# Meeso1/nmmo

Hardware: AMD Instinct MI355X
Metric: agent-steps/sec (whole node), 128-agent envs at 1/2/4/8 MI355X (higher is better)
Workload: dtype int16

## Files before the change

nmmo_amd/csrc/flat_obs.hip:

```cpp
#include "agent_obs.h"

namespace nmmo {

#ifndef NMMO_FO_ABL
#define NMMO_FO_ABL 0
#endif
#ifndef NMMO_FO_STAMPS
#define NMMO_FO_STAMPS 0
#endif
#if NMMO_FO_STAMPS
constexpr int kFoStamps = 12;
__device__ uint64_t fo_stamp_buf[1 << 17][kFoStamps];
__device__ uint64_t fo_wave_buf[1 << 15][6];
#define FO_STAMP(k) fst[k] = __builtin_amdgcn_s_memtime()
#else
#define FO_STAMP(k) (void)0
#endif
#ifndef NMMO_FO_XCD
#define NMMO_FO_XCD 1
#endif
#ifndef NMMO_FO_TILE_SKIP
#define NMMO_FO_TILE_SKIP 0
#endif
#ifndef NMMO_FO_TASK_BATCH
#define NMMO_FO_TASK_BATCH 8
#endif
constexpr int kFoTaskBatch = NMMO_FO_TASK_BATCH;
constexpr int kFoStagedListings = 64;
constexpr int kFoChunks = 25;
static_assert(kFoChunks * 64 >= kMaskN + 2 && (kFoChunks - 1) * 64 < kMaskN, "mask chunks");
static_assert(kFlatId == kMaskN && kFlatTick == kMaskN + 1 && kFlatEntity == kMaskN + 2, "id, tick in the last chunk");
static_assert(kWireBuyLo / 64 == 1 && (kWireBuyLo + NMMO_MARKET_ROWS) / 64 == 17, "Buy.MarketItem: chunks 1 to 17");

constexpr int kFoVisw = (kNObs + 3) & ~3;
constexpr int kFoWinRowBytes = 16, kFoWinAgentBytes = 15 * kFoWinRowBytes;
constexpr size_t kFoWinBytes = (size_t)kAoAgents * kFoWinAgentBytes, kFoItemBytes = (size_t)kAoAgents * kInv * 8;
static_assert(F_COL == F_ROW + 1 && kAoPkBytes <= kFoWinBytes, "shared LDS regions");
__host__ __device__ constexpr bool fo_items_in_T(int S) {
  return (size_t)2 * ao_stride(S) * 2 >= kFoItemBytes && (F_ROW * ao_stride(S) * 2) % 8 == 0;
}
constexpr int kFoListPool = NMMO_MARKET_ROWS * 2 + kFoStagedListings * 8;
__host__ __device__ constexpr int fo_staged(int nm) {
  return nm < ((kFoListPool - ((2 * nm + 7) & ~7)) >> 3) ? nm : (kFoListPool - ((2 * nm + 7) & ~7)) >> 3;
}
static_assert(fo_staged(NMMO_MARKET_ROWS) == kFoStagedListings && fo_staged(256) == 256 && fo_staged(257) == 255 &&
                  fo_staged(0) == 0 && kFoListPool % 16 == 0, "listings' pool");
__host__ __device__ constexpr size_t fo_lds_bytes(int S) {
  return ao_columns_lds(S) + (size_t)kFoListPool +
         (size_t)kAoWaves * kFoVisw * 4 + kFoWinBytes + (fo_items_in_T(S) ? 0 : kFoItemBytes);
// ... 17 lines not shown
__device__ __forceinline__ uint64_t fo_shift(uint64_t lo, uint64_t hi) {
  if constexpr (kSh >= 64) {
    return 0ull;
  } else if constexpr (kSh > 0) {
    return lo << kSh;
  } else if constexpr (kSh == 0) {
    return lo;
  } else if constexpr (-kSh < 64) {
    return (lo >> (-kSh)) | (hi << (64 + kSh));
  } else if constexpr (-kSh < 128) {
    return hi >> (-kSh - 64);
  } else {
    return 0ull;
  }
}
template <int kK, int kC>
__device__ __forceinline__ uint64_t fo_sec(uint64_t lo, uint64_t hi) {
  constexpr int off = sec_flat(kK), n = kSecN[kK];
  if constexpr (off >= 64 * kC + 64 || off + n <= 64 * kC) return 0ull;
  else return fo_shift<off - 64 * kC>(lo, hi);
}
template <int kC>
__device__ __forceinline__ uint64_t fo_chunk(const AoSections& x) {
  return fo_sec<0, kC>(x.s0, 0ull) | fo_sec<1, kC>(x.s1[0], x.s1[1]) | fo_sec<3, kC>(x.s3, 0ull) |
         fo_sec<4, kC>(x.s4, 0ull) | fo_sec<5, kC>(x.s5[0], x.s5[1]) | fo_sec<6, kC>(x.s6[0], x.s6[1]) |
         fo_sec<7, kC>(x.s7[0], x.s7[1]) | fo_sec<8, kC>(x.s8, 0ull) | fo_sec<9, kC>(x.s9, 0ull) |
         fo_sec<10, kC>(x.s10[0], x.s10[1]) | fo_sec<11, kC>(x.s11, 0ull);
}
__device__ __forceinline__ float fo_bit(uint64_t m) { return __builtin_amdgcn_inverse_ballot_w64(m) ? 1.f : 0.f; }
__device__ __forceinline__ void fo_st(float* row, uint32_t idx, float v) {
  *reinterpret_cast<float*>(reinterpret_cast<char*>(row) + (idx << 2)) = v;
}

constexpr int kFoTail0 = (kWireBuyLo + NMMO_MARKET_ROWS) / 64;
__host__ __device__ constexpr int fo_slot(int c) { return c < 2 ? c : c - kFoTail0 + 2; }
static_assert(fo_slot(kFoChunks - 1) == 9 && kZext == 10 + 1 + 12, "tracked chunks | position | items");
struct FoImg {
  bool ext;
  uint32_t lo, hi;
  int j10;
  int nimg;
  int nst;
};
__device__ __forceinline__ uint64_t fo_prev(const FoImg& g, int slot) {
  return (uint64_t)(uint32_t)__builtin_amdgcn_readlane((int)g.lo, g.j10 + slot) |
         (uint64_t)(uint32_t)__builtin_amdgcn_readlane((int)g.hi, g.j10 + slot) << 32;
}
template <int kC>
__device__ __forceinline__ void fo_put(float* row, FoImg& g, uint64_t m, float aid, float tick) {
  constexpr int sl = fo_slot(kC);
  const int lane = ao_lane();
  const bool same = g.ext && m == fo_prev(g, sl);
  if constexpr (kC == kFoChunks - 1) {
    constexpr int n = kMaskN - 64 * kC;
    if (!same) {
      if (lane < n + 2) fo_st(row, 64 * kC + lane, lane < n ? fo_bit(m) : lane == n ? aid : tick);
      g.nst += n + 2;
    } else {
      if (lane == n + 1) fo_st(row, 64 * kC + lane, tick);
      g.nst += 1;
    }
  } else if (!same) {
    fo_st(row, 64 * kC + lane, fo_bit(m));
    g.nst += 64;
  }
  g.nimg = writelane<2 * sl>((int)(uint32_t)m, g.nimg);
  g.nimg = writelane<2 * sl + 1>((int)(uint32_t)(m >> 32), g.nimg);
}
template <int kC>
__device__ __forceinline__ void fo_tail_chunks(float* row, FoImg& g, const AoSections& x, uint64_t buy17, float aid,
                                               float tick) {
  if constexpr (kC < kFoChunks) {
    uint64_t m = fo_chunk<kC>(x);
    if constexpr (kC == kFoTail0) m |= buy17 | 1ull << ((kWireBuyLo + NMMO_MARKET_ROWS) & 63);
    fo_put<kC>(row, g, m, aid, tick);
    fo_tail_chunks<kC + 1>(row, g, x, buy17, aid, tick);
  }
}

constexpr int kFoPassRows = 16;
static_assert(kFoPassRows == 16 && kAoAgents / kAoWaves * kFoPassRows <= 64 && kInv <= kFoPassRows &&
                  kFoGather <= kFoPassRows, "a 16-lane group per agent");
constexpr int kFoBuyLane = 48;
struct FoPass {
  uint32_t lo, hi;
  uint64_t chg;
  uint64_t idiff;
};
template <int kSl>
__device__ __forceinline__ void fo_pass_chunks(const AoSections& x, int sl, uint64_t& m) {
  if constexpr (kSl < 10) {
    constexpr int c = kSl < 2 ? kSl : kSl - 2 + kFoTail0;
    static_assert(fo_slot(c) == kSl, "tracked chunk");
    const uint64_t mc = fo_chunk<c>(x);
    if (sl == kSl) m = mc;
    fo_pass_chunks<kSl + 1>(x, sl, m);
  }
}
template <bool kWrap>
__device__ __forceinline__ FoPass fo_mask_pass(const ObsParams& p, int e, int w, int abase, int nm, const int16_t* own,
                                               const uint32_t* visw, const uint8_t* wsb, const uint2* ist,
                                               const uint16_t* mpo, int my_nv, uint32_t my_rc, int my_prev, int my_alive,
                                               int my_task, uint64_t zvalid, uint64_t zextv, uint2 img, uint2 pinv) {
  constexpr int kPerWave = kAoAgents / kAoWaves;
  const bool combat = (p.systems & NMMO_SYS_COMBAT) != 0;
  const bool item = (p.systems & NMMO_SYS_ITEM) != 0;
  const bool exch = item && (p.systems & NMMO_SYS_EXCHANGE) != 0;
  const bool no_give = kWrap && (p.wflags & kWrapObsNoGive);
  const bool no_danger = kWrap && (p.wflags & kWrapObsNoDangerous);
  const int lane = lane_id(), P = p.P;
  const int gj = lane >> 4, gk = lane & 15, ga = abase + kAoWaves * gj, gla = w + kAoWaves * gj;
  const int grc = __shfl((int)my_rc, gj);
  const int gr = (int16_t)(grc & 0xFFFF), gc = grc >> 16;
  bool tgt = false, st = false;
  if (gk < __shfl(my_nv, gj)) ao_row_preds(visw[gj * kFoVisw + gk], ga, gr, gc, combat, no_danger, tgt, st);
  const uint64_t tb = __ballot(tgt), sb = __ballot(st);
  const uint2 it = gk < kInv ? ist[gla * kInv + gk] : make_uint2(0u, 0u);
  const uint64_t occ = __ballot(gk < kInv && it_type(it) != 0);
  const bool have = gk < __builtin_ctz(~((uint32_t)(occ >> (16 * gj)) & 0xFFFFu));
  const uint64_t bfr = __ballot(have && !it_equipped(it) && !it_price(it));
// ... 64 lines not shown
#pragma unroll
    for (int d = 0; d < 5; d++)
      if (!impassable((int)wa[(kVision + dir_dr(d)) * kFoWinRowBytes + kVision + dir_dc(d)])) b |= 1u << d;
    x.s8 = b;
  }
  uint64_t m = 0ull;
  fo_pass_chunks<0>(x, sl, m);
  uint64_t bw0 = 0ull, bw15 = 0ull;
  FoPass o;
  o.lo = img.x;
  o.hi = img.y;
  if (exch && nm > 0) {
    const uint32_t po0 = lane < nm ? mpo[lane] : 0u, po15 = 15 * 64 + lane < nm ? mpo[15 * 64 + lane] : 0u;
#pragma unroll
    for (int j = 0; j < kPerWave; j++) {
      const int a = abase + kAoWaves * j;
      const int gold = __builtin_amdgcn_readfirstlane((int)own[(w + kAoWaves * j) * kMirrorCols + F_GOLD]);
      const uint64_t b0 = __ballot(lane < nm && (int)(po0 & 255u) <= gold && (int)(po0 >> 8) != a);
      uint64_t b15 = 0ull;
      if (nm > 15 * 64) b15 = __ballot(15 * 64 + lane < nm && (int)(po15 & 255u) <= gold && (int)(po15 >> 8) != a);
      if (ja == j) bw0 = b0, bw15 = b15;
      if (lane == kFoBuyLane + j) o.lo = (uint32_t)b0, o.hi = (uint32_t)(b0 >> 32);
    }
  }
  if (sl == 1) m |= bw0 << (kWireBuyLo & 63);
  if (sl == 2) m |= bw15 >> (64 - (kWireBuyLo & 63)) | 1ull << ((kWireBuyLo + NMMO_MARKET_ROWS) & 63);
  const bool ext = (zextv >> ja) & 1;
  o.chg = __ballot(lane < 10 * kPerWave && (!ext || (uint32_t)m != img.x || (uint32_t)(m >> 32) != img.y));
  if (lane < 10 * kPerWave) o.lo = (uint32_t)m, o.hi = (uint32_t)(m >> 32);
  const int ji = min(lane / kInv, kPerWave - 1);
  const uint2 iw = ist[(w + kAoWaves * ji) * kInv + lane % kInv];
  const bool idl = lane < kInv * kPerWave && (!((zextv >> ji) & 1) || iw.x != pinv.x || iw.y != pinv.y);
  o.idiff = __ballot(idl);
  {
    const int jp = lane < 10 * kPerWave ? ja : min(lane - 10 * kPerWave, kPerWave - 1);
    const size_t ai = (size_t)e * P + min(abase + kAoWaves * jp, P - 1);
    uint2 wv = make_uint2(o.lo, o.hi);
    const int rcp = __shfl((int)my_rc, jp);
    if (lane >= 10 * kPerWave) {
      wv = make_uint2((uint32_t)((int)(int16_t)(rcp & 0xFFFF) | (rcp >> 16) << 8), 0u);
    }
    const int alp = __shfl(my_alive, jp);
    if (lane < 11 * kPerWave && alp) reinterpret_cast<uint2*>(p.zext)[ai * kZext + (lane < 10 * kPerWave ? sl : 10)] = wv;
    const size_t ii = (size_t)e * P + min(abase + kAoWaves * ji, P - 1);
    const int ali = __shfl(my_alive, ji);
    if (idl && ali) reinterpret_cast<uint2*>(p.zext)[ii * kZext + 11 + lane % kInv] = iw;
    if (lane < kPerWave && my_alive) {
      const size_t am = (size_t)e * P + abase + kAoWaves * lane;
      if (!((zvalid >> lane) & 1)) p.zrow[am] = p.ztag;
      p.zst[am] = zs_pack((my_nv + 1) & ~1, nm, my_task) | kZsExt;
    }
  }
  return o;
}

struct IcDesc {
  uint32_t tmA, tmB;
  uint32_t f;
};
__device__ __forceinline__ IcDesc ic_desc(int col) {
  auto bits = [](int lo, int hi) { return ((2u << hi) - 1u) & ~((1u << lo) - 1u); };
  IcDesc d{0u, 0u, 0u};
  auto bf = [&](int sel, int sh, int wd) { d.f = (uint32_t)(sel | sh << 1 | wd << 6); };
  switch (col) {
    case 0: bf(1, 16, 16); break;
    case 1: bf(0, 0, 5); break;
// ... 38 lines not shown
    nvis += __popcll(b);
  }
  return nvis;
}

typedef const __attribute__((address_space(4))) ObsParams* FoArgs;

template <bool kWrap, int kS, bool kAligned = true, bool kMirror = false>
__global__ void __launch_bounds__(64 * kAoWaves) __attribute__((amdgpu_waves_per_eu(5, 5))) flat_obs_kernel(ObsParams p) {
  static_assert(!kMirror || (kS == kMaxSlots && kAligned), "the mirror variant: 384 slots");
  extern __shared__ __attribute__((aligned(16))) unsigned char smem[];
  const int S = kS ? kS : p.S, P = p.P, Sp = ao_stride(S), tdim = p.task_dim, elems = kFlatTask + tdim + kTileN;
  constexpr int kPerWave = kAoAgents / kAoWaves;
  static_assert(!kMirror || (kPerWave * kFoGather) % 16 == 0, "gather: 16 rows per load instruction");
  int16_t* T = reinterpret_cast<int16_t*>(smem);
  int16_t* gat = reinterpret_cast<int16_t*>(smem + kFoOwnBytes);
  uint16_t* mpo = reinterpret_cast<uint16_t*>(smem + (kMirror ? kFoOwnBytes + kFoGatBytes : ao_columns_lds(S)));
  uint32_t* visw_all = reinterpret_cast<uint32_t*>(mpo) + kFoListPool / 4;
  uint2* mtop = reinterpret_cast<uint2*>(visw_all) - 1;
  uint32_t* wst = visw_all + (kMirror ? kAoAgents : kAoWaves) * kFoVisw;
  uint32_t* pk = wst;
  uint2* ist = reinterpret_cast<uint2*>(!kMirror && fo_items_in_T(S) ? smem + (size_t)F_ROW * Sp * 2
                                                                     : reinterpret_cast<unsigned char*>(wst) + kFoWinBytes);
#if NMMO_FO_XCD
  int el, g;
  ao_env_group(p.env_list ? p.n_list : p.n_envs, (p.P + kAoAgents - 1) / kAoAgents, el, g);
#else
  const int el = blockIdx.x, g = blockIdx.y;
#endif
  const int e = p.env_list ? p.env_list[el] : el, tid = threadIdx.x, lane = lane_id();
  if ((unsigned)e >= (unsigned)p.n_envs) return;
  if (NMMO_FO_ABL & 128) return;
#if NMMO_FO_STAMPS
  uint64_t wst_[6];
  wst_[0] = __builtin_amdgcn_s_memtime();
#endif
  const int w = __builtin_amdgcn_readfirstlane(wave_id());
  AoStage sg;
  const int16_t* M = kMirror ? p.frows + (size_t)e * S * kMirrorCols : nullptr;
  uint32_t pr[kAoRows];
  uint4 ow = make_uint4(0u, 0u, 0u, 0u);
  int wpr = 0, wpc = 0;
  if constexpr (kMirror) {
    sg.nm = p.mcount[e];
    sg.mv = p.mlist[(size_t)e * NMMO_MARKET_ROWS + min(tid, NMMO_MARKET_ROWS - 1)];
#pragma unroll
    for (int i = 0; i < kAoRows; i++) pr[i] = p.fpk[(size_t)e * kMaxSlots + lane + 64 * i];
    ow = reinterpret_cast<const uint4*>(M + (size_t)min(g * kAoAgents + ((tid >> 2) & (kAoAgents - 1)), P - 1) * kMirrorCols)[tid & 3];
    const int16_t* wr = M + (size_t)min(g * kAoAgents + tid / 15, P - 1) * kMirrorCols;
    wpr = wr[F_ROW];
    wpc = wr[F_COL];
  } else {
    ao_stage_load<kAligned>(p, e, sg);
  }
  const int16_t* E = p.ent + (size_t)e * NMMO_NF * S;
  const int abase = g * kAoAgents + w;
  int my_task = 0, my_prev = -1, my_alive = 0;
  uint64_t my_z = 0, my_s = 0;
  const bool mine = lane < kPerWave && abase + kAoWaves * lane < P;
  {
    const int aj = min(abase + kAoWaves * min(lane, kPerWave - 1), P - 1);
    const size_t ai = (size_t)e * P + aj;
    my_task = p.assign[ai];
    my_alive = kMirror ? M[(size_t)aj * kMirrorCols + kMirrorCols - 1] : E[F_ALIVE * S + aj];
    if (p.zrow) {
      my_z = p.zrow[ai];
      my_s = p.zst[ai];
// ... 77 lines not shown
  const int nm = min(max(sg.nm, 0), NMMO_MARKET_ROWS), nst = fo_staged(nm);
  const uint2 lwd = ao_listing_load(p, e, sg);
  auto listings = [&]() {
    if constexpr (kMirror) {
      uint4* gd = reinterpret_cast<uint4*>(gat) + w * kGatIt * 64 + lane;
      gd[0] = gq0;
      if constexpr (kGatIt > 1) gd[64] = gq1;
      if constexpr (kGatIt > 2) gd[128] = gq2;
      if constexpr (kGatIt > 3) gd[192] = gq3;
    }
    if (tid < nm) {
      mpo[tid] = (uint16_t)(it_price(lwd) | ((sg.mv >> 16) & 255) << 8);
      if (tid < nst) mtop[-tid] = lwd;
    }
    for (int j = tid + (int)blockDim.x; j < nm; j += blockDim.x) {
      const int v = p.mlist[(size_t)e * NMMO_MARKET_ROWS + j];
      const int own = (v >> 16) & 255, slot = (v >> 24) & 15;
      const uint2 wd = p.items[((size_t)e * P + own) * kInv + slot];
      mpo[j] = (uint16_t)(it_price(wd) | own << 8);
      if (j < nst) mtop[-j] = wd;
    }
  };
  if constexpr (kMirror)
    ao_stage_windows_at<kAoAgents, kFoWinRowBytes / 4, true>(p, e, g, wpr, wpc, wst, ist, listings);
  else
    ao_stage_windows<kAoAgents, kFoWinRowBytes / 4>(p, e, g, T, Sp, wst, ist, listings, []() { __syncthreads(); });
#if NMMO_FO_STAMPS
  wst_[2] = __builtin_amdgcn_s_memtime();
#endif
  asm volatile("" : "+v"(img.x), "+v"(img.y), "+v"(pinv.x), "+v"(pinv.y), "+v"(my_prev));
  if (!img_ok) img = make_uint2(0u, 0u);
  if (!pinv_ok) pinv = make_uint2(0u, 0u);
  const int my_h = !zvl ? (kNObs | NMMO_MARKET_ROWS << 12) : zzl ? 0 : (zs_hv(my_s) | zs_hm(my_s) << 12);
  FoPass mp{img.x, img.y, ~0ull, ~0ull};
  if constexpr (kMirror) {
    if (!(NMMO_FO_ABL & 1))
      mp = fo_mask_pass<kWrap>(p, e, w, abase, nm, T, visw, wsb, ist, mpo, my_nv, my_rc, my_prev, my_alive, my_task, zvalid,
                               zextv, img, pinv);
  }
  int nrows = 0;
  unsigned long long nbytes = 0;
  int wo[2];
  ao_win_offsets<kFoWinRowBytes>(wo);
  int toff[4];
#pragma unroll
  for (int i = 0; i < 4; i++) {
    const int t = lane + 64 * i;
    toff[i] = ((t / 15 - kVision) & 255) | (t % 15 - kVision) * 256;
  }
  const int ef = lane & 31, eh = lane >> 5;
  const int iq = lane >> 4;
  const IcDesc icd = ic_desc(lane & 15);

#if NMMO_FO_STAMPS
  wst_[3] = __builtin_amdgcn_s_memtime();
#endif
#pragma unroll 1
  for (int j = 0; j < ((NMMO_FO_ABL & 64) ? 0 : kPerWave); j++) {
    const int a = abase + kAoWaves * j;
    if (a >= P) break;
    const int lane = ao_lane();
    FoArgs kp = (FoArgs)__builtin_amdgcn_kernarg_segment_ptr();
    asm volatile("" : "+s"(kp));
    auto grow = (__attribute__((address_space(1))) float*)(p.obs + ((NMMO_FO_ABL & 256)
        ? (size_t)(((e * P + a) & 15) + 16 * (blockIdx.x & 7)) : (size_t)e * P + a) * elems);
    asm volatile("" : "+s"(grow));
    float* row = (float*)grow;
    const bool zv = (zvalid >> j) & 1;
    const int hj = __builtin_amdgcn_readlane(my_h, j);
    const int hv = hj & 4095, hm = hj >> 12;
    if (!__builtin_amdgcn_readlane(my_alive, j)) {
      if ((zzero >> j) & 1) {
        if ((ztile >> j) & 1) {
          wave_zero(row, kFlatTask + tdim, elems);
          nbytes += 4ull * (elems - kFlatTask - tdim);
          if (lane == 0) kp->zst[(size_t)e * P + a] = kZsZero;
          nrows++;
        }
        continue;
      }
      if (zv) {
        wave_zero(row, 0, kFlatEntity + hv * NMMO_N_ENTITY_COLS);
        wave_zero(row, kFlatInv, kFlatMarket + hm * 16);
        wave_zero(row, kFlatTask, elems);
        nbytes += 4ull * (kFlatEntity + hv * NMMO_N_ENTITY_COLS + kFlatMarket + hm * 16 - kFlatInv + elems - kFlatTask);
      } else {
        wave_zero(row, 0, elems);
        nbytes += 4ull * elems;
      }
      if (lane == 0) {
        kp->zrow[(size_t)e * P + a] = kp->ztag;
        kp->zst[(size_t)e * P + a] = kZsZero;
      }
      nrows++;
      continue;
    }
    nrows++;
#if NMMO_FO_STAMPS
    uint64_t fst[kFoStamps];
#endif
    FO_STAMP(0);
    const int la = a - g * kAoAgents;
    const int rcj = __builtin_amdgcn_readlane((int)my_rc, j);
    const int r = (int16_t)(rcj & 0xFFFF), c = rcj >> 16;
    const int16_t* Ta = kMirror ? T + la * kMirrorCols : T;
    const int Spa = kMirror ? 1 : Sp, tia = kMirror ? 0 : a;
    if constexpr (kMirror) visw = visw_all + (w * kPerWave + j) * kFoVisw;
    const int gold = __builtin_amdgcn_readfirstlane(Ta[F_GOLD * Spa + tia]);
    const int aid = __builtin_amdgcn_readfirstlane(Ta[F_ID * Spa + tia]);
    const uint8_t* wa = wsb + la * kFoWinAgentBytes;
    uint32_t wm[4];
#pragma unroll
    for (int i = 0; i < 4; i++) wm[i] = lane + 64 * i < 225 ? wa[ao_win_off(wo, i)] : 0u;
    uint2 it = make_uint2(0u, 0u);
    uint32_t mv = 0u;
    int ninv = 0;
    if constexpr (!kMirror) {
      it = lane < kInv ? ist[la * kInv + lane] : make_uint2(0u, 0u);
      mv = ao_move_bits(wm[1]);
      ninv = __builtin_ctzll(~__ballot(lane < kInv && it_type(it) != 0));
    }
    int nv;
    if constexpr (kMirror) {
      nv = __builtin_amdgcn_readlane(my_nv, j);
    } else {
      nv = (NMMO_FO_ABL & 32) ? 0 : min(fo_compact(pr, r, c, visw), kNObs);
      __builtin_amdgcn_fence(__ATOMIC_RELEASE, "wavefront");
      __builtin_amdgcn_wave_barrier();
      __builtin_amdgcn_fence(__ATOMIC_ACQUIRE, "wavefront");
    }

    FO_STAMP(1);
    const bool ext = (zextv >> j) & 1;
    FoImg fg{ext, img.x, img.y, 10 * j, 0, 0};
    if constexpr (kMirror) {
      if (!(NMMO_FO_ABL & 1)) {
        const uint32_t chg = (uint32_t)(mp.chg >> (10 * j)) & 0x3FFu;
        auto pm = [&](int l) {
          return (uint64_t)(uint32_t)__builtin_amdgcn_readlane((int)mp.lo, l) |
                 (uint64_t)(uint32_t)__builtin_amdgcn_readlane((int)mp.hi, l) << 32;
        };
        int nst = 0;
        FO_STAMP(2);
#pragma unroll 1
        for (uint32_t cs = chg & 3u; cs; cs &= cs - 1u) {
          const int s = __builtin_ctz(cs);
          fo_st(row, 64 * s + lane, fo_bit(pm(10 * j + s)));
          nst += 64;
        }
        FO_STAMP(3);
        auto buy_word = [&](int m) {
          const int k = 64 * m + lane;
          bool bv = false;
          if (exch && k < nm) {
            const uint32_t po = mpo[k];
            bv = (int)(po & 255u) <= gold && (int)(po >> 8) != a;
          }
          return __ballot(bv);
        };
        const int clast = max(1, min((kWireBuyLo + max(nm, hm) - 1) >> 6, 16));
        uint64_t bprev = pm(kFoBuyLane + j);
#pragma unroll 1
        for (int cc = 2; cc <= clast; cc++) {
          const uint64_t bcur = 64 * (cc - 1) < nm ? buy_word(cc - 1) : 0ull;
          fo_st(row, 64 * cc + lane, fo_bit(bcur << (kWireBuyLo & 63) | bprev >> (64 - (kWireBuyLo & 63))));
          bprev = bcur;
        }
        FO_STAMP(4);
#pragma unroll 1
        for (uint32_t cs = (chg >> 2) & 0x7Fu; cs; cs &= cs - 1u) {
          const int s = __builtin_ctz(cs);
          fo_st(row, 64 * (kFoTail0 + s) + lane, fo_bit(pm(10 * j + 2 + s)));
          nst += 64;
        }
        constexpr int kc = kFoChunks - 1, n = kMaskN - 64 * kc;
        if (chg >> 9) {
          const uint64_t m = pm(10 * j + 9);
          if (lane < n + 2) fo_st(row, 64 * kc + lane, lane < n ? fo_bit(m) : lane == n ? (float)aid : tickf);
          nst += n + 2;
        } else {
          if (lane == n + 1) fo_st(row, 64 * kc + lane, tickf);
          nst += 1;
        }
        nbytes += 4ull * (nst + 64 * (clast - 1));
      }
    } else if (!(NMMO_FO_ABL & 1)) {
      AoAgent ag;
      ag.a = a;
      ag.ti = tia;
      ag.r = r;
      ag.c = c;
      ag.gold = gold;
      ag.aid = aid;
      ag.nv = nv;
      ag.ninv = ninv;
      ag.prev_price = kWrap ? __builtin_amdgcn_readlane(my_prev, j) : -1;
      ag.mv = mv;
      const AoSections x = ao_sections<kWrap>(p, Ta, Spa, visw, ag, it);
      FO_STAMP(2);
      fg.ext = ext;
      fo_put<0>(row, fg, fo_chunk<0>(x), 0.f, 0.f);
      auto buy_word = [&](int m) {
        const int k = 64 * m + lane;
        bool bv = false;
        if (exch && k < nm) {
          const uint32_t po = mpo[k];
          bv = (int)(po & 255u) <= gold && (int)(po >> 8) != a;
        }
        return __ballot(bv);
      };
      const int nbuy = max(nm, hm);
      const int clast = max(1, min((kWireBuyLo + nbuy - 1) >> 6, 16));
      uint64_t bprev = nm > 0 ? buy_word(0) : 0ull;
      fo_put<1>(row, fg, fo_chunk<1>(x) | bprev << (kWireBuyLo & 63), 0.f, 0.f);
      FO_STAMP(3);
#pragma unroll 1
      for (int cc = 2; cc <= clast; cc++) {
        const uint64_t bcur = 64 * (cc - 1) < nm ? buy_word(cc - 1) : 0ull;
        fo_st(row, 64 * cc + lane, fo_bit(bcur << (kWireBuyLo & 63) | bprev >> (64 - (kWireBuyLo & 63))));
        bprev = bcur;
      }
      FO_STAMP(4);
      const uint64_t buy17 = nm > 15 * 64 ? bprev >> (64 - (kWireBuyLo & 63)) : 0ull;
      fo_tail_chunks<kFoTail0>(row, fg, x, buy17, (float)aid, tickf);
      nbytes += 4ull * (fg.nst + 64 * (clast - 1));
    }
    FO_STAMP(5);
    const int nv2 = (nv + 1) & ~1;
    if (!(NMMO_FO_ABL & 2)) {
      const uint32_t de = kFlatEntity + (lane - eh);
      const bool epos = (lane & 31) == F_ROW || (lane & 31) == F_COL;
      const uint32_t esh = (lane & 31) == F_COL ? 16u : 0u;
      const int16_t* gj = gat + (size_t)(w * kPerWave + j) * kFoGather * kMirrorCols;
      const int nst2 = kMirror ? min(nv2, kFoGather) : nv2;
#pragma unroll 1
      for (int k0 = 0; k0 < nst2; k0 += 2) {
        const int k = k0 + eh;
        if (ef < NMMO_N_ENTITY_COLS) {
          float v = 0.f;
          if (k < nv) {
            const uint32_t vw = visw[k];
            const int tv = kMirror ? gj[k * kMirrorCols + ef] : T[ef * Sp + ao_slot(vw)];
            v = (float)(epos ? (int)((vw >> esh) & 255u) : tv);
          }
          fo_st(row, de + k0 * NMMO_N_ENTITY_COLS, v);
        }
      }
      if constexpr (kMirror) {
        if (nv2 > kFoGather) {
          const int16_t* Mk = kp->frows + (size_t)e * kMaxSlots * kMirrorCols;
#pragma unroll 1
          for (int k0 = kFoGather; k0 < nv2; k0 += 2) {
            const int k = k0 + eh;
            if (ef < NMMO_N_ENTITY_COLS) {
              float v = 0.f;
              if (k < nv) {
                const uint32_t vw = visw[k];
                const int tv = Mk[(size_t)min(ao_slot(vw), kMaxSlots - 1) * kMirrorCols + ef];
                v = (float)(epos ? (int)((vw >> esh) & 255u) : tv);
              }
              fo_st(row, de + k0 * NMMO_N_ENTITY_COLS, v);
            }
          }
        }
      }
      const int hz = max(nv2, hv);
      wave_zero(row, kFlatEntity + nv2 * NMMO_N_ENTITY_COLS, kFlatEntity + hz * NMMO_N_ENTITY_COLS);
      nbytes += 4ull * (hz * NMMO_N_ENTITY_COLS + max(nm, hm) * 16);
    }
    FO_STAMP(6);
    bool inv_same;
    if constexpr (kMirror) {
      inv_same = ((uint32_t)(mp.idiff >> (kInv * j)) & ((1u << kInv) - 1u)) == 0u;
    } else {
      const int jl = (12 * j + lane) & 63;
      const uint32_t px = (uint32_t)__shfl((int)pinv.x, jl), py = (uint32_t)__shfl((int)pinv.y, jl);
      inv_same = ext && __ballot(lane < kInv && (px != it.x || py != it.y)) == 0ull;
    }
    if (!inv_same) {
      if constexpr (kMirror) ninv = __builtin_ctzll(~__ballot(lane < kInv && it_type(ist[la * kInv + min(lane, kInv - 1)]) != 0));
#pragma unroll
      for (int h = 0; h < ((NMMO_FO_ABL & 4) ? 0 : kInv * 16 / 64); h++) {
        const int q = 4 * h + iq;
        float v = 0.f;
        if (4 * h < ninv && q < ninv) v = ic_value(ist[la * kInv + q], aid, icd);
        fo_st(row, kFlatInv + 64 * h + lane, v);
      }
      nbytes += 4ull * kInv * 16;
    }
    FO_STAMP(7);
    const int nms = (NMMO_FO_ABL & 8) ? 0 : fo_staged(nm);
    for (int k = lane; k < nms * 16; k += 64) fo_st(row, kFlatMarket + k, ic_value(mtop[-(k >> 4)], (mpo[k >> 4] >> 8) + 1, icd));
    if (nm > nms && !(NMMO_FO_ABL & 8)) {
      for (int k = nms * 16 + lane; k < nm * 16; k += 64) {
        const int q = k >> 4;
        const int v = kp->mlist[(size_t)e * NMMO_MARKET_ROWS + q];
        const uint2 wd = kp->items[((size_t)e * P + ((v >> 16) & 255)) * kInv + ((v >> 24) & 15)];
        fo_st(row, kFlatMarket + k, ic_value(wd, (mpo[q] >> 8) + 1, icd));
      }
    }
    wave_zero(row, kFlatMarket + nm * 16, kFlatMarket + max(nm, hm) * 16);
    FO_STAMP(8);
    const int task = __builtin_amdgcn_readlane(my_task, j);
    if (!((ztask >> j) & 1)) {
      const float* temb = kp->task + (size_t)task * tdim;
      int k0 = 0;
      for (; k0 + kFoTaskBatch * 64 <= tdim; k0 += kFoTaskBatch * 64) {
        float t[kFoTaskBatch];
#pragma unroll
        for (int i = 0; i < kFoTaskBatch; i++) t[i] = temb[k0 + 64 * i + lane];
#pragma unroll
        for (int i = 0; i < kFoTaskBatch; i++) fo_st(row, kFlatTask + k0 + 64 * i + lane, t[i]);
      }
      for (int k = k0 + lane; k < tdim; k += 64) fo_st(row, kFlatTask + k, temb[k]);
      nbytes += 4ull * tdim;
    }
    FO_STAMP(9);
    const uint32_t ppos = (uint32_t)__builtin_amdgcn_readlane((int)(kMirror ? mp.lo : img.x), 40 + j);
    const bool tkn = NMMO_FO_TILE_SKIP && ext && !((ztile >> j) & 1);
    const bool same_r = tkn && (int)(ppos & 255u) == r, same_c = tkn && (int)((ppos >> 8) & 255u) == c;
    if (!(NMMO_FO_ABL & 16)) {
      float* dt = row + kFlatTask + tdim + 3 * lane;
#pragma unroll
      for (int i = 0; i < 4; i++) {
        if (lane + 64 * i < 225) {
          const float vr = (float)(r + ((toff[i] << 24) >> 24)), vc = (float)(c + (toff[i] >> 8)), vm = (float)wm[i];
          if (NMMO_FO_TILE_SKIP) {
            if (!same_r) dt[192 * i] = vr;
            if (!same_c) dt[192 * i + 1] = vc;
            dt[192 * i + 2] = vm;
          } else {
            typedef float f3 __attribute__((ext_vector_type(3)));
            const f3 v = {vr, vc, vm};
            __builtin_memcpy(dt + 192 * i, &v, 12);
          }
        }
      }
      nbytes += 4ull * 225 * (1 + !same_r + !same_c);
    }
    FO_STAMP(10);
    if constexpr (!kMirror) {
      uint32_t* zx = reinterpret_cast<uint32_t*>(kp->zext + ((size_t)e * P + a) * kZext);
      int wv = fg.nimg;
      if (lane == 20) wv = r | c << 8;
      if (lane == 21) wv = 0;
      if (lane < 22) zx[lane] = (uint32_t)wv;
      if (!inv_same && lane < kInv) reinterpret_cast<uint2*>(zx + 22)[lane] = it;
      if (lane == 0) {
        if (!zv) kp->zrow[(size_t)e * P + a] = kp->ztag;
        kp->zst[(size_t)e * P + a] = zs_pack(nv2, nm, task) | kZsExt;
      }
    }
#if NMMO_FO_STAMPS
    FO_STAMP(11);
    if (lane == 0 && (size_t)e * P + a < (1u << 17))
      for (int k = 0; k < kFoStamps; k++) fo_stamp_buf[(size_t)e * P + a][k] = fst[k];
#endif
    if constexpr (!kMirror) {
      __builtin_amdgcn_fence(__ATOMIC_RELEASE, "wavefront");
      __builtin_amdgcn_wave_barrier();
      __builtin_amdgcn_fence(__ATOMIC_ACQUIRE, "wavefront");
    }
  }
#if NMMO_FO_STAMPS
  wst_[4] = __builtin_amdgcn_s_memtime();
  wst_[5] = (uint64_t)e | (uint64_t)nrows << 32;
  {
    const size_t wi = ((size_t)blockIdx.y * gridDim.x + blockIdx.x) * kAoWaves + w;
    if (lane == 0 && wi < (1u << 15))
      for (int k = 0; k < 6; k++) fo_wave_buf[wi][k] = wst_[k];
  }
#endif
  if (p.rows_out && lane == 0 && nrows) {
    atomicAdd(&p.rows_out[2 * e], (unsigned long long)nrows);
    atomicAdd(&p.rows_out[2 * e + 1], nbytes);
  }
}

hipError_t launch_flat_obs(const ObsParams& p, hipStream_t stream) {
  if (!(p.obs && p.ztag && p.zrow)) return hipErrorInvalidValue;
  const int ne = list_grid(p.env_list, p.n_list, p.n_envs);
  if (ne <= 0) return hipSuccess;
#if NMMO_FO_XCD
  const dim3 grid(ne * ((p.P + kAoAgents - 1) / kAoAgents)), block(64 * kAoWaves);
#else
  const dim3 grid(ne, (p.P + kAoAgents - 1) / kAoAgents), block(64 * kAoWaves);
#endif
  const size_t lds = fo_lds_bytes(p.S);
  if (p.frows) {
    if (!p.fpk || !p.zext || p.S != kMaxSlots) return hipErrorInvalidValue;
    if (p.wflags) hipLaunchKernelGGL((flat_obs_kernel<true, kMaxSlots, true, true>), grid, block, kFoMirrorLds, stream, p);
    else hipLaunchKernelGGL((flat_obs_kernel<false, kMaxSlots, true, true>), grid, block, kFoMirrorLds, stream, p);
  } else if (p.S == kMaxSlots) {
    if (p.wflags) hipLaunchKernelGGL((flat_obs_kernel<true, kMaxSlots>), grid, block, lds, stream, p);
    else hipLaunchKernelGGL((flat_obs_kernel<false, kMaxSlots>), grid, block, lds, stream, p);
  } else if (p.S % 8 != 0) {
    if (p.wflags) hipLaunchKernelGGL((flat_obs_kernel<true, 0, false>), grid, block, lds, stream, p);
    else hipLaunchKernelGGL((flat_obs_kernel<false, 0, false>), grid, block, lds, stream, p);
  } else {
    if (p.wflags) hipLaunchKernelGGL((flat_obs_kernel<true, 0>), grid, block, lds, stream, p);
    else hipLaunchKernelGGL((flat_obs_kernel<false, 0>), grid, block, lds, stream, p);
  }
  return hipGetLastError();
// ... 23 lines not shown
```

Baseline: 381.3 million.

## Restructure mirror flat-obs writer into phase-major loops across a wave's agents

In the mirror path, the per-agent loop that wrote every section of one agent's row before moving to the next is replaced by phase-major passes. Each section (mask, entities, inventory, market, task, tile window) is now written for all live agents of the wave in one pass. Shared values such as market item encodings and LDS loads are computed once and stored to every agent's row, and entity gathers for all four agents are batched per step. This aims to cut redundant recomputation and improve memory-level parallelism, at the cost of more live registers and a much larger, more complex code path. The mask pass also exports inventory occupancy, and the timing-stamp buffer is widened.

```diff
diff --git a/nmmo_amd/csrc/flat_obs.hip b/nmmo_amd/csrc/flat_obs.hip
--- a/nmmo_amd/csrc/flat_obs.hip
+++ b/nmmo_amd/csrc/flat_obs.hip
@@ -11,10 +11,13 @@
 #if NMMO_FO_STAMPS
 constexpr int kFoStamps = 12;
 __device__ uint64_t fo_stamp_buf[1 << 17][kFoStamps];
-__device__ uint64_t fo_wave_buf[1 << 15][6];
+constexpr int kFoWaveStamps = 12;
+__device__ uint64_t fo_wave_buf[1 << 15][kFoWaveStamps];
 #define FO_STAMP(k) fst[k] = __builtin_amdgcn_s_memtime()
+#define FO_WSTAMP(k) wst_[k] = __builtin_amdgcn_s_memtime()
 #else
 #define FO_STAMP(k) (void)0
+#define FO_WSTAMP(k) (void)0
 #endif
 #ifndef NMMO_FO_XCD
 #define NMMO_FO_XCD 1
@@ -98,6 +101,12 @@
   *reinterpret_cast<float*>(reinterpret_cast<char*>(row) + (idx << 2)) = v;
 }
 
+__device__ __forceinline__ void fo_st3(float* row, uint32_t idx, float a, float b, float c) {
+  typedef float f3 __attribute__((ext_vector_type(3)));
+  const f3 v = {a, b, c};
+  __builtin_memcpy(reinterpret_cast<char*>(row) + (idx << 2), &v, 12);
+}
+
 constexpr int kFoTail0 = (kWireBuyLo + NMMO_MARKET_ROWS) / 64;
 __host__ __device__ constexpr int fo_slot(int c) { return c < 2 ? c : c - kFoTail0 + 2; }
 static_assert(fo_slot(kFoChunks - 1) == 9 && kZext == 10 + 1 + 12, "tracked chunks | position | items");
@@ -152,6 +161,7 @@
   uint32_t lo, hi;
   uint64_t chg;
   uint64_t idiff;
+  uint64_t occ;
 };
 template <int kSl>
 __device__ __forceinline__ void fo_pass_chunks(const AoSections& x, int sl, uint64_t& m) {
@@ -282,6 +292,7 @@
   const uint2 iw = ist[(w + kAoWaves * ji) * kInv + lane % kInv];
   const bool idl = lane < kInv * kPerWave && (!((zextv >> ji) & 1) || iw.x != pinv.x || iw.y != pinv.y);
   o.idiff = __ballot(idl);
+  o.occ = occ;
   {
     const int jp = lane < 10 * kPerWave ? ja : min(lane - 10 * kPerWave, kPerWave - 1);
     const size_t ai = (size_t)e * P + min(abase + kAoWaves * jp, P - 1);
@@ -386,7 +397,7 @@
   if ((unsigned)e >= (unsigned)p.n_envs) return;
   if (NMMO_FO_ABL & 128) return;
 #if NMMO_FO_STAMPS
-  uint64_t wst_[6];
+  uint64_t wst_[kFoWaveStamps] = {};
   wst_[0] = __builtin_amdgcn_s_memtime();
 #endif
   const int w = __builtin_amdgcn_readfirstlane(wave_id());
@@ -530,7 +541,7 @@
   if (!img_ok) img = make_uint2(0u, 0u);
   if (!pinv_ok) pinv = make_uint2(0u, 0u);
   const int my_h = !zvl ? (kNObs | NMMO_MARKET_ROWS << 12) : zzl ? 0 : (zs_hv(my_s) | zs_hm(my_s) << 12);
-  FoPass mp{img.x, img.y, ~0ull, ~0ull};
+  FoPass mp{img.x, img.y, ~0ull, ~0ull, 0ull};
   if constexpr (kMirror) {
     if (!(NMMO_FO_ABL & 1))
       mp = fo_mask_pass<kWrap>(p, e, w, abase, nm, T, visw, wsb, ist, mpo, my_nv, my_rc, my_prev, my_alive, my_task, zvalid,
@@ -553,6 +564,298 @@
 #if NMMO_FO_STAMPS
   wst_[3] = __builtin_amdgcn_s_memtime();
 #endif
+  if constexpr (kMirror) {
+    typedef __attribute__((address_space(1))) float* FoRow;
+    auto rowp = [&](int j) {
+      auto grow = (FoRow)(p.obs + ((NMMO_FO_ABL & 256) ? (size_t)(((e * P + abase + kAoWaves * j) & 15) + 16 * (blockIdx.x & 7))
+                                                       : (size_t)e * P + abase + kAoWaves * j) * elems);
+      asm volatile("" : "+s"(grow));
+      return (float*)grow;
+    };
+    auto kargs = []() {
+      FoArgs kp = (FoArgs)__builtin_amdgcn_kernarg_segment_ptr();
+      asm volatile("" : "+s"(kp));
+      return kp;
+    };
+    uint32_t live = 0u;
+#pragma unroll 1
+    for (int j = 0; j < ((NMMO_FO_ABL & 64) ? 0 : kPerWave); j++) {
+      const int a = abase + kAoWaves * j;
+      if (a >= P) break;
+      if (__builtin_amdgcn_readlane(my_alive, j)) {
+        live |= 1u << j;
+        nrows++;
+        continue;
+      }
+      const int lane = ao_lane();
+      FoArgs kp = kargs();
+      float* row = rowp(j);
+      if ((zzero >> j) & 1) {
+        if ((ztile >> j) & 1) {
+          wave_zero(row, kFlatTask + tdim, elems);
+          nbytes += 4ull * (elems - kFlatTask - tdim);
+          if (lane == 0) kp->zst[(size_t)e * P + a] = kZsZero;
+          nrows++;
+        }
+        continue;
+      }
+      if ((zvalid >> j) & 1) {
+        const int hj = __builtin_amdgcn_readlane(my_h, j);
+        const int hv = hj & 4095, hm = hj >> 12;
+        wave_zero(row, 0, kFlatEntity + hv * NMMO_N_ENTITY_COLS);
+        wave_zero(row, kFlatInv, kFlatMarket + hm * 16);
+        wave_zero(row, kFlatTask, elems);
+        nbytes += 4ull * (kFlatEntity + hv * NMMO_N_ENTITY_COLS + kFlatMarket + hm * 16 - kFlatInv + elems - kFlatTask);
+      } else {
+        wave_zero(row, 0, elems);
+        nbytes += 4ull * elems;
+      }
+      if (lane == 0) {
+        kp->zrow[(size_t)e * P + a] = kp->ztag;
+        kp->zst[(size_t)e * P + a] = kZsZero;
+      }
+      nrows++;
+    }
+    FO_WSTAMP(4);
+    float* rows[kPerWave];
+#pragma unroll
+    for (int j = 0; j < kPerWave; j++) rows[j] = rowp(j);
+    if (!(NMMO_FO_ABL & 1)) {
+#pragma unroll 1
+      for (int j = 0; j < kPerWave; j++) {
+        if (!((live >> j) & 1)) continue;
+        const int lane = ao_lane();
+        const int a = abase + kAoWaves * j;
+        float* row = rowp(j);
+        const int16_t* Ta = T + (w + kAoWaves * j) * kMirrorCols;
+        const int gold = __builtin_amdgcn_readfirstlane(Ta[F_GOLD]);
+        const int aid = __builtin_amdgcn_readfirstlane(Ta[F_ID]);
+        const int hm = __builtin_amdgcn_readlane(my_h, j) >> 12;
+        const uint32_t chg = (uint32_t)(mp.chg >> (10 * j)) & 0x3FFu;
+        auto pm = [&](int l) {
+          return (uint64_t)(uint32_t)__builtin_amdgcn_readlane((int)mp.lo, l) |
+                 (uint64_t)(uint32_t)__builtin_amdgcn_readlane((int)mp.hi, l) << 32;
+        };
+        int nst = 0;
+#pragma unroll 1
+        for (uint32_t cs = chg & 3u; cs; cs &= cs - 1u) {
+          const int s = __builtin_ctz(cs);
+          fo_st(row, 64 * s + lane, fo_bit(pm(10 * j + s)));
+          nst += 64;
+        }
+        auto buy_word = [&](int m) {
+          const int k = 64 * m + lane;
+          bool bv = false;
+          if (exch && k < nm) {
+            const uint32_t po = mpo[k];
+            bv = (int)(po & 255u) <= gold && (int)(po >> 8) != a;
+          }
+          return __ballot(bv);
+        };
+        const int clast = max(1, min((kWireBuyLo + max(nm, hm) - 1) >> 6, 16));
+        uint64_t bprev = pm(kFoBuyLane + j);
+#pragma unroll 1
+        for (int cc = 2; cc <= clast; cc++) {
+          const uint64_t bcur = 64 * (cc - 1) < nm ? buy_word(cc - 1) : 0ull;
+          fo_st(row, 64 * cc + lane, fo_bit(bcur << (kWireBuyLo & 63) | bprev >> (64 - (kWireBuyLo & 63))));
+          bprev = bcur;
+        }
+#pragma unroll 1
+        for (uint32_t cs = (chg >> 2) & 0x7Fu; cs; cs &= cs - 1u) {
+          const int s = __builtin_ctz(cs);
+          fo_st(row, 64 * (kFoTail0 + s) + lane, fo_bit(pm(10 * j + 2 + s)));
+          nst += 64;
+        }
+        constexpr int kc = kFoChunks - 1, n = kMaskN - 64 * kc;
+        if (chg >> 9) {
+          const uint64_t m = pm(10 * j + 9);
+          if (lane < n + 2) fo_st(row, 64 * kc + lane, lane < n ? fo_bit(m) : lane == n ? (float)aid : tickf);
+          nst += n + 2;
+        } else {
+          if (lane == n + 1) fo_st(row, 64 * kc + lane, tickf);
+          nst += 1;
+        }
+        nbytes += 4ull * (nst + 64 * (clast - 1));
+      }
+    }
+    FO_WSTAMP(5);
+    if (!(NMMO_FO_ABL & 2)) {
+      const int lane = ao_lane();
+      const int ef = lane & 31, eh = lane >> 5;
+      const uint32_t de = kFlatEntity + (lane - eh);
+      const bool epos = ef == F_ROW || ef == F_COL;
+      const uint32_t esh = ef == F_COL ? 16u : 0u;
+      const int16_t* gw = gat + (size_t)(w * kPerWave) * kFoGather * kMirrorCols;
+      int nvs[kPerWave], nst2[kPerWave], kmax = 0;
+#pragma unroll
+      for (int j = 0; j < kPerWave; j++) {
+        nvs[j] = ((live >> j) & 1) ? __builtin_amdgcn_readlane(my_nv, j) : 0;
+        nst2[j] = min((nvs[j] + 1) & ~1, kFoGather);
+        kmax = max(kmax, nst2[j]);
+      }
+#pragma unroll 1
+      for (int k0 = 0; k0 < kmax; k0 += 2) {
+        const int k = k0 + eh;
+        uint32_t vw[kPerWave];
+        int tv[kPerWave];
+#pragma unroll
+        for (int j = 0; j < kPerWave; j++) vw[j] = visw[j * kFoVisw + k];
+#pragma unroll
+        for (int j = 0; j < kPerWave; j++) tv[j] = gw[(j * kFoGather + k) * kMirrorCols + ef];
+        asm volatile("" : "+v"(vw[0]), "+v"(vw[1]), "+v"(vw[2]), "+v"(vw[3]), "+v"(tv[0]), "+v"(tv[1]), "+v"(tv[2]), "+v"(tv[3]));
+#pragma unroll
+        for (int j = 0; j < kPerWave; j++) {
+          if (k0 < nst2[j]) {
+            const float v = k < nvs[j] ? (float)(epos ? (int)((vw[j] >> esh) & 255u) : tv[j]) : 0.f;
+            if (ef < NMMO_N_ENTITY_COLS) fo_st(rows[j], de + k0 * NMMO_N_ENTITY_COLS, v);
+          }
+        }
+      }
+#pragma unroll 1
+      for (int j = 0; j < kPerWave; j++) {
+        if (!((live >> j) & 1)) continue;
+        float* row = rowp(j);
+        const int nv = __builtin_amdgcn_readlane(my_nv, j), nv2 = (nv + 1) & ~1;
+        const int hj = __builtin_amdgcn_readlane(my_h, j);
+        const int hv = hj & 4095, hm = hj >> 12;
+        if (nv2 > kFoGather) {
+          const int16_t* Mk = kargs()->frows + (size_t)e * kMaxSlots * kMirrorCols;
+#pragma unroll 1
+          for (int k0 = kFoGather; k0 < nv2; k0 += 2) {
+            const int k = k0 + eh;
+            if (ef < NMMO_N_ENTITY_COLS) {
+              float v = 0.f;
+              if (k < nv) {
+                const uint32_t vwk = visw[j * kFoVisw + k];
+                const int tvk = Mk[(size_t)min(ao_slot(vwk), kMaxSlots - 1) * kMirrorCols + ef];
+                v = (float)(epos ? (int)((vwk >> esh) & 255u) : tvk);
+              }
+              fo_st(row, de + k0 * NMMO_N_ENTITY_COLS, v);
+            }
+          }
+        }
+        const int hz = max(nv2, hv);
+        if (hz > nv2) wave_zero(row, kFlatEntity + nv2 * NMMO_N_ENTITY_COLS, kFlatEntity + hz * NMMO_N_ENTITY_COLS);
+        nbytes += 4ull * (hz * NMMO_N_ENTITY_COLS + max(nm, hm) * 16);
+      }
+    }
+    FO_WSTAMP(6);
+    if (!(NMMO_FO_ABL & 4)) {
+      uint32_t wr = 0u;
+#pragma unroll
+      for (int j = 0; j < kPerWave; j++)
+        if (((live >> j) & 1) && ((uint32_t)(mp.idiff >> (kInv * j)) & ((1u << kInv) - 1u))) wr |= 1u << j;
+      if (wr) {
+        const int lane = ao_lane();
+        const int iq = lane >> 4;
+        uint2 iw[kPerWave][kInv * 16 / 64];
+        int aid[kPerWave];
+#pragma unroll
+        for (int j = 0; j < kPerWave; j++) {
+#pragma unroll
+          for (int h = 0; h < kInv * 16 / 64; h++) iw[j][h] = ist[(w + kAoWaves * j) * kInv + 4 * h + iq];
+          aid[j] = T[(w + kAoWaves * j) * kMirrorCols + F_ID];
+        }
+#pragma unroll
+        for (int j = 0; j < kPerWave; j++) {
+          if ((wr >> j) & 1) {
+            const int ninv = __builtin_ctz(~((uint32_t)(mp.occ >> (16 * j)) & 0xFFFFu));
+#pragma unroll
+            for (int h = 0; h < kInv * 16 / 64; h++) {
+              const float v = 4 * h + iq < ninv ? ic_value(iw[j][h], aid[j], icd) : 0.f;
+              fo_st(rows[j], kFlatInv + 64 * h + lane, v);
+            }
+            nbytes += 4ull * kInv * 16;
+          }
+        }
+      }
+    }
+    FO_WSTAMP(7);
+    if (!(NMMO_FO_ABL & 8) && live) {
+      const int lane = ao_lane();
+      const int nms = fo_staged(nm);
+      for (int k = lane; k < nms * 16; k += 64) {
+        const float v = ic_value(mtop[-(k >> 4)], (mpo[k >> 4] >> 8) + 1, icd);
+#pragma unroll
+        for (int j = 0; j < kPerWave; j++)
+          if ((live >> j) & 1) fo_st(rows[j], kFlatMarket + k, v);
+      }
+      if (nm > nms) {
+        FoArgs kp = kargs();
+        for (int k = nms * 16 + lane; k < nm * 16; k += 64) {
+          const int q = k >> 4;
+          const int lv = kp->mlist[(size_t)e * NMMO_MARKET_ROWS + q];
+          const uint2 wd = kp->items[((size_t)e * P + ((lv >> 16) & 255)) * kInv + ((lv >> 24) & 15)];
+          const float v = ic_value(wd, (mpo[q] >> 8) + 1, icd);
+#pragma unroll
+          for (int j = 0; j < kPerWave; j++)
+            if ((live >> j) & 1) fo_st(rows[j], kFlatMarket + k, v);
+        }
+      }
+#pragma unroll 1
+      for (int j = 0; j < kPerWave; j++) {
+        const int hm = __builtin_amdgcn_readlane(my_h, j) >> 12;
+        if (((live >> j) & 1) && hm > nm) wave_zero(rowp(j), kFlatMarket + nm * 16, kFlatMarket + hm * 16);
+      }
+    }
+    FO_WSTAMP(8);
+    if (live & ~(uint32_t)ztask) {
+#pragma unroll 1
+      for (int j = 0; j < kPerWave; j++) {
+        if (!((live >> j) & 1) || ((ztask >> j) & 1)) continue;
+        const int lane = ao_lane();
+        float* row = rowp(j);
+        const float* temb = kargs()->task + (size_t)__builtin_amdgcn_readlane(my_task, j) * tdim;
+        int k0 = 0;
+        for (; k0 + kFoTaskBatch * 64 <= tdim; k0 += kFoTaskBatch * 64) {
+          float t[kFoTaskBatch];
+#pragma unroll
+          for (int i = 0; i < kFoTaskBatch; i++) t[i] = temb[k0 + 64 * i + lane];
+#pragma unroll
+          for (int i = 0; i < kFoTaskBatch; i++) fo_st(row, kFlatTask + k0 + 64 * i + lane, t[i]);
+        }
+        for (int k = k0 + lane; k < tdim; k += 64) fo_st(row, kFlatTask + k, temb[k]);
+        nbytes += 4ull * tdim;
+      }
+    }
+    FO_WSTAMP(9);
+    if (!(NMMO_FO_ABL & 16)) {
+      const int lane = ao_lane();
+      const uint32_t dt = kFlatTask + tdim + 3 * lane;
+      uint32_t wm[kPerWave][4];
+#pragma unroll
+      for (int j = 0; j < kPerWave; j++) {
+        const uint8_t* wa = wsb + (w + kAoWaves * j) * kFoWinAgentBytes;
+#pragma unroll
+        for (int i = 0; i < 4; i++) wm[j][i] = wa[ao_win_off(wo, i)];
+      }
+#pragma unroll
+      for (int j = 0; j < kPerWave; j++) {
+        if ((live >> j) & 1) {
+          const int rcj = __builtin_amdgcn_readlane((int)my_rc, j);
+          const int r = (int16_t)(rcj & 0xFFFF), c = rcj >> 16;
+          const uint32_t ppos = (uint32_t)__builtin_amdgcn_readlane((int)mp.lo, 40 + j);
+          const bool tkn = NMMO_FO_TILE_SKIP && ((zextv >> j) & 1) && !((ztile >> j) & 1);
+          const bool same_r = tkn && (int)(ppos & 255u) == r, same_c = tkn && (int)((ppos >> 8) & 255u) == c;
+#pragma unroll
+          for (int i = 0; i < 4; i++) {
+            if (i < 3 || lane < 225 - 192) {
+              const float vr = (float)(r + ((toff[i] << 24) >> 24)), vc = (float)(c + (toff[i] >> 8)), vm = (float)wm[j][i];
+              if (NMMO_FO_TILE_SKIP) {
+                if (!same_r) fo_st(rows[j], dt + 192 * i, vr);
+                if (!same_c) fo_st(rows[j], dt + 192 * i + 1, vc);
+                fo_st(rows[j], dt + 192 * i + 2, vm);
+              } else {
+                fo_st3(rows[j], dt + 192 * i, vr, vc, vm);
+              }
+            }
+          }
+          nbytes += 4ull * 225 * (1 + !same_r + !same_c);
+        }
+      }
+    }
+  }
+  if constexpr (!kMirror)
 #pragma unroll 1
   for (int j = 0; j < ((NMMO_FO_ABL & 64) ? 0 : kPerWave); j++) {
     const int a = abase + kAoWaves * j;
@@ -601,88 +904,26 @@
     const int la = a - g * kAoAgents;
     const int rcj = __builtin_amdgcn_readlane((int)my_rc, j);
     const int r = (int16_t)(rcj & 0xFFFF), c = rcj >> 16;
-    const int16_t* Ta = kMirror ? T + la * kMirrorCols : T;
-    const int Spa = kMirror ? 1 : Sp, tia = kMirror ? 0 : a;
-    if constexpr (kMirror) visw = visw_all + (w * kPerWave + j) * kFoVisw;
+    const int16_t* Ta = T;
+    const int Spa = Sp, tia = a;
     const int gold = __builtin_amdgcn_readfirstlane(Ta[F_GOLD * Spa + tia]);
     const int aid = __builtin_amdgcn_readfirstlane(Ta[F_ID * Spa + tia]);
     const uint8_t* wa = wsb + la * kFoWinAgentBytes;
     uint32_t wm[4];
 #pragma unroll
     for (int i = 0; i < 4; i++) wm[i] = lane + 64 * i < 225 ? wa[ao_win_off(wo, i)] : 0u;
-    uint2 it = make_uint2(0u, 0u);
-    uint32_t mv = 0u;
-    int ninv = 0;
-    if constexpr (!kMirror) {
-      it = lane < kInv ? ist[la * kInv + lane] : make_uint2(0u, 0u);
-      mv = ao_move_bits(wm[1]);
-      ninv = __builtin_ctzll(~__ballot(lane < kInv && it_type(it) != 0));
-    }
-    int nv;
-    if constexpr (kMirror) {
-      nv = __builtin_amdgcn_readlane(my_nv, j);
-    } else {
-      nv = (NMMO_FO_ABL & 32) ? 0 : min(fo_compact(pr, r, c, visw), kNObs);
-      __builtin_amdgcn_fence(__ATOMIC_RELEASE, "wavefront");
-      __builtin_amdgcn_wave_barrier();
-      __builtin_amdgcn_fence(__ATOMIC_ACQUIRE, "wavefront");
-    }
+    const uint2 it = lane < kInv ? ist[la * kInv + lane] : make_uint2(0u, 0u);
+    const uint32_t mv = ao_move_bits(wm[1]);
+    const int ninv = __builtin_ctzll(~__ballot(lane < kInv && it_type(it) != 0));
+    const int nv = (NMMO_FO_ABL & 32) ? 0 : min(fo_compact(pr, r, c, visw), kNObs);
+    __builtin_amdgcn_fence(__ATOMIC_RELEASE, "wavefront");
+    __builtin_amdgcn_wave_barrier();
+    __builtin_amdgcn_fence(__ATOMIC_ACQUIRE, "wavefront");
 
     FO_STAMP(1);
     const bool ext = (zextv >> j) & 1;
     FoImg fg{ext, img.x, img.y, 10 * j, 0, 0};
-    if constexpr (kMirror) {
-      if (!(NMMO_FO_ABL & 1)) {
-        const uint32_t chg = (uint32_t)(mp.chg >> (10 * j)) & 0x3FFu;
-        auto pm = [&](int l) {
-          return (uint64_t)(uint32_t)__builtin_amdgcn_readlane((int)mp.lo, l) |
-                 (uint64_t)(uint32_t)__builtin_amdgcn_readlane((int)mp.hi, l) << 32;
-        };
-        int nst = 0;
-        FO_STAMP(2);
-#pragma unroll 1
-        for (uint32_t cs = chg & 3u; cs; cs &= cs - 1u) {
-          const int s = __builtin_ctz(cs);
-          fo_st(row, 64 * s + lane, fo_bit(pm(10 * j + s)));
-          nst += 64;
-        }
-        FO_STAMP(3);
-        auto buy_word = [&](int m) {
-          const int k = 64 * m + lane;
-          bool bv = false;
-          if (exch && k < nm) {
-            const uint32_t po = mpo[k];
-            bv = (int)(po & 255u) <= gold && (int)(po >> 8) != a;
-          }
-          return __ballot(bv);
-        };
-        const int clast = max(1, min((kWireBuyLo + max(nm, hm) - 1) >> 6, 16));
-        uint64_t bprev = pm(kFoBuyLane + j);
-#pragma unroll 1
-        for (int cc = 2; cc <= clast; cc++) {
-          const uint64_t bcur = 64 * (cc - 1) < nm ? buy_word(cc - 1) : 0ull;
-          fo_st(row, 64 * cc + lane, fo_bit(bcur << (kWireBuyLo & 63) | bprev >> (64 - (kWireBuyLo & 63))));
-          bprev = bcur;
-        }
-        FO_STAMP(4);
-#pragma unroll 1
-        for (uint32_t cs = (chg >> 2) & 0x7Fu; cs; cs &= cs - 1u) {
-          const int s = __builtin_ctz(cs);
-          fo_st(row, 64 * (kFoTail0 + s) + lane, fo_bit(pm(10 * j + 2 + s)));
-          nst += 64;
-        }
-        constexpr int kc = kFoChunks - 1, n = kMaskN - 64 * kc;
-        if (chg >> 9) {
-          const uint64_t m = pm(10 * j + 9);
-          if (lane < n + 2) fo_st(row, 64 * kc + lane, lane < n ? fo_bit(m) : lane == n ? (float)aid : tickf);
-          nst += n + 2;
-        } else {
-          if (lane == n + 1) fo_st(row, 64 * kc + lane, tickf);
-          nst += 1;
-        }
-        nbytes += 4ull * (nst + 64 * (clast - 1));
-      }
-    } else if (!(NMMO_FO_ABL & 1)) {
+    if (!(NMMO_FO_ABL & 1)) {
       AoAgent ag;
       ag.a = a;
       ag.ti = tia;
@@ -729,54 +970,28 @@
       const uint32_t de = kFlatEntity + (lane - eh);
       const bool epos = (lane & 31) == F_ROW || (lane & 31) == F_COL;
       const uint32_t esh = (lane & 31) == F_COL ? 16u : 0u;
-      const int16_t* gj = gat + (size_t)(w * kPerWave + j) * kFoGather * kMirrorCols;
-      const int nst2 = kMirror ? min(nv2, kFoGather) : nv2;
-#pragma unroll 1
-      for (int k0 = 0; k0 < nst2; k0 += 2) {
+#pragma unroll 1
+      for (int k0 = 0; k0 < nv2; k0 += 2) {
         const int k = k0 + eh;
         if (ef < NMMO_N_ENTITY_COLS) {
           float v = 0.f;
           if (k < nv) {
             const uint32_t vw = visw[k];
-            const int tv = kMirror ? gj[k * kMirrorCols + ef] : T[ef * Sp + ao_slot(vw)];
+            const int tv = T[ef * Sp + ao_slot(vw)];
             v = (float)(epos ? (int)((vw >> esh) & 255u) : tv);
           }
           fo_st(row, de + k0 * NMMO_N_ENTITY_COLS, v);
         }
       }
-      if constexpr (kMirror) {
-        if (nv2 > kFoGather) {
-          const int16_t* Mk = kp->frows + (size_t)e * kMaxSlots * kMirrorCols;
-#pragma unroll 1
-          for (int k0 = kFoGather; k0 < nv2; k0 += 2) {
-            const int k = k0 + eh;
-            if (ef < NMMO_N_ENTITY_COLS) {
-              float v = 0.f;
-              if (k < nv) {
-                const uint32_t vw = visw[k];
-                const int tv = Mk[(size_t)min(ao_slot(vw), kMaxSlots - 1) * kMirrorCols + ef];
-                v = (float)(epos ? (int)((vw >> esh) & 255u) : tv);
-              }
-              fo_st(row, de + k0 * NMMO_N_ENTITY_COLS, v);
-            }
-          }
-        }
-      }
       const int hz = max(nv2, hv);
       wave_zero(row, kFlatEntity + nv2 * NMMO_N_ENTITY_COLS, kFlatEntity + hz * NMMO_N_ENTITY_COLS);
       nbytes += 4ull * (hz * NMMO_N_ENTITY_COLS + max(nm, hm) * 16);
     }
     FO_STAMP(6);
-    bool inv_same;
-    if constexpr (kMirror) {
-      inv_same = ((uint32_t)(mp.idiff >> (kInv * j)) & ((1u << kInv) - 1u)) == 0u;
-    } else {
-      const int jl = (12 * j + lane) & 63;
-      const uint32_t px = (uint32_t)__shfl((int)pinv.x, jl), py = (uint32_t)__shfl((int)pinv.y, jl);
-      inv_same = ext && __ballot(lane < kInv && (px != it.x || py != it.y)) == 0ull;
-    }
+    const int jl = (12 * j + lane) & 63;
+    const uint32_t px = (uint32_t)__shfl((int)pinv.x, jl), py = (uint32_t)__shfl((int)pinv.y, jl);
+    const bool inv_same = ext && __ballot(lane < kInv && (px != it.x || py != it.y)) == 0ull;
     if (!inv_same) {
-      if constexpr (kMirror) ninv = __builtin_ctzll(~__ballot(lane < kInv && it_type(ist[la * kInv + min(lane, kInv - 1)]) != 0));
 #pragma unroll
       for (int h = 0; h < ((NMMO_FO_ABL & 4) ? 0 : kInv * 16 / 64); h++) {
         const int q = 4 * h + iq;
@@ -814,7 +1029,7 @@
       nbytes += 4ull * tdim;
     }
     FO_STAMP(9);
-    const uint32_t ppos = (uint32_t)__builtin_amdgcn_readlane((int)(kMirror ? mp.lo : img.x), 40 + j);
+    const uint32_t ppos = (uint32_t)__builtin_amdgcn_readlane((int)img.x, 40 + j);
     const bool tkn = NMMO_FO_TILE_SKIP && ext && !((ztile >> j) & 1);
     const bool same_r = tkn && (int)(ppos & 255u) == r, same_c = tkn && (int)((ppos >> 8) & 255u) == c;
     if (!(NMMO_FO_ABL & 16)) {
@@ -837,7 +1052,7 @@
       nbytes += 4ull * 225 * (1 + !same_r + !same_c);
     }
     FO_STAMP(10);
-    if constexpr (!kMirror) {
+    {
       uint32_t* zx = reinterpret_cast<uint32_t*>(kp->zext + ((size_t)e * P + a) * kZext);
       int wv = fg.nimg;
       if (lane == 20) wv = r | c << 8;
@@ -854,19 +1069,17 @@
     if (lane == 0 && (size_t)e * P + a < (1u << 17))
       for (int k = 0; k < kFoStamps; k++) fo_stamp_buf[(size_t)e * P + a][k] = fst[k];
 #endif
-    if constexpr (!kMirror) {
-      __builtin_amdgcn_fence(__ATOMIC_RELEASE, "wavefront");
-      __builtin_amdgcn_wave_barrier();
-      __builtin_amdgcn_fence(__ATOMIC_ACQUIRE, "wavefront");
-    }
+    __builtin_amdgcn_fence(__ATOMIC_RELEASE, "wavefront");
+    __builtin_amdgcn_wave_barrier();
+    __builtin_amdgcn_fence(__ATOMIC_ACQUIRE, "wavefront");
   }
 #if NMMO_FO_STAMPS
-  wst_[4] = __builtin_amdgcn_s_memtime();
-  wst_[5] = (uint64_t)e | (uint64_t)nrows << 32;
+  wst_[kFoWaveStamps - 2] = __builtin_amdgcn_s_memtime();
+  wst_[kFoWaveStamps - 1] = (uint64_t)e | (uint64_t)nrows << 32;
   {
     const size_t wi = ((size_t)blockIdx.y * gridDim.x + blockIdx.x) * kAoWaves + w;
     if (lane == 0 && wi < (1u << 15))
-      for (int k = 0; k < 6; k++) fo_wave_buf[wi][k] = wst_[k];
+      for (int k = 0; k < kFoWaveStamps; k++) fo_wave_buf[wi][k] = wst_[k];
   }
 #endif
   if (p.rows_out && lane == 0 && nrows) {
```

Result: no change. 383.4 million (median of 6 runs) (+0.6%).
